# lgleznah/mort

Measured on AMD Instinct MI355X. Metric: Msamples/sec (width x height x spp/s), Scene 1 1200x675, higher is better.
Workload: dtype f32; 1 GPU; Scene 1 (random-spheres cover) 1200x675, 500 spp nominal = 484 effective, depth 20, megakernel, seed 69420, host LCG scene; mode=mega, partition=rows/8 interleaved over 1 rank(s)

## Files before the change

### mort_amd/csrc/hip/dev_scene.h

```cpp
#ifndef MORT_DEV_SCENE_H
#define MORT_DEV_SCENE_H

#include <stdint.h>
#include "mort_scene.h"

#define DREF(type, idx) (((uint32_t)(type) << 16) | (uint32_t)(idx))
#define DREF_TYPE(r) ((int)((r) >> 16) & 0x7fff)
#define DREF_IDX(r) ((int)((r) & 0xffffu))

struct __attribute__((aligned(16))) DSphere {
    float cx, cy, cz, radius;
    float vx, vy, vz;
    uint32_t mat;
};

struct __attribute__((aligned(16))) DQuad {
    float Q[3], D;
    float u[3], area;
    float v[3]; uint32_t mat;
    float n[3]; uint32_t pad0;
    float w[3]; uint32_t pad1;
};

struct __attribute__((aligned(16))) DBvhNode {
    float xmin, xmax, ymin, ymax, zmin, zmax;
    uint32_t skip;
    uint32_t prims;
};

struct __attribute__((aligned(16))) DNode2 {
    float x0min, x0max, y0min, y0max;
    float z0min, z0max, x1min, x1max;
    float y1min, y1max, z1min, z1max;
    uint32_t child0, child1;
    float e0, e1;
};
struct __attribute__((aligned(16))) DNode4 {
    float xmin[4], xmax[4], ymin[4], ymax[4], zmin[4], zmax[4], e[4];
    uint32_t child[4];
    uint32_t pad[4];
};
struct __attribute__((aligned(16))) DLeaf2 {
    DSphere a, b;
    float xmin, xmax, ymin, ymax, zmin, zmax;
    uint32_t n;
    uint32_t prims;
    uint32_t pad[4];
};
#define MORT_NODE4_PIECES 9
#define MORT_LEAF2_PIECES 7
#define MORT_OWN4_STACK 24
struct __attribute__((aligned(16))) DNodeQ {
    float ox, oy, oz;
    uint32_t exps;
    uint32_t q0;
    uint32_t q1;
    uint32_t q2;
    uint32_t children;
};
#define GLEAF_FIRST(ref) ((ref) & 0x1fffu)
#define GLEAF_COUNT(ref) ((((ref) >> 13) & 3u) + 1u)
#define MORT_OWN_STACK 16
#define MORT_OWN_MAX_DEPTH 15
#ifndef MORT_GEN_LEAF_MAX
#define MORT_GEN_LEAF_MAX 2
#endif
#define GENT(kind, chain, idx) (((uint32_t)(kind) << 31) | ((uint32_t)(chain) << 24) | (uint32_t)(idx))
#define GENT_QUAD(e) ((e) >> 31)
#define GENT_CHAIN(e) (((e) >> 24) & 0x7fu)
#define GENT_IDX(e) ((e) & 0xffffffu)

enum { XF_TRANSLATE = 0, XF_ROTATE_Y = 1 };
// ... 47 lines not shown
```

### mort_amd/csrc/hip/mega_bvh.h

```cpp
#ifndef MORT_MEGA_BVH_H
#define MORT_MEGA_BVH_H

#include "dev_render.h"


struct FastArgs {
    RenderArgs r;
    const unsigned char *hot_src;
    uint32_t hot_bytes;
    uint32_t off_nodes4, off_leafrecs, off_lambert, off_metal, off_diel, off_dlight, off_iso, off_solid, off_checker;
    uint32_t off_tstack;
    int node_first, node_count;
    unsigned int *next_q;
    int tiles_x, tiles_total;
    uint32_t off_stack;
    int stack_lds_depth;
    const unsigned *tile_order;
    int gen_tiles;
    int spread_shift;
    unsigned *tile_cost;
    int th_s, th_l, t_keep;
    int sub;
    float *vaccum;
    float4 *deep;
// ... 12 lines not shown
#define MORT_BVH_ARG_NAME
#endif
#ifdef MORT_BVH_NO_PIN
#define BU_I(x) (x)
#define BU_U(x) (x)
#define BU_F(x) (x)
#define BU_P(x) (x)
#else
#define BU_I(x) uni_i(x)
#define BU_U(x) uni_u(x)
#define BU_F(x) uni_f(x)
#define BU_P(x) uni_p(x)
#endif
__device__ __forceinline__ int uni_i(int x) { return __builtin_amdgcn_readfirstlane(x); }
__device__ __forceinline__ uint32_t uni_u(uint32_t x) { return (uint32_t)__builtin_amdgcn_readfirstlane((int)x); }
__device__ __forceinline__ float uni_f(float x) { return __int_as_float(__builtin_amdgcn_readfirstlane(__float_as_int(x))); }
template <typename T> __device__ __forceinline__ T *uni_p(T *p) {
    const unsigned long long v = (unsigned long long)p;
    const uint32_t lo = uni_u((uint32_t)v), hi = uni_u((uint32_t)(v >> 32));
    return (T *)(((unsigned long long)hi << 32) | (unsigned long long)lo);
}

enum { ST_T = 0, ST_L = 1, ST_S = 2, ST_DONE = 3 };
enum { FL_TIE = 1, FL_REF = 2 };
#ifdef MORT_REGION_MARKS
#define REGION(name) asm volatile("; REGION " name)
#else
#define REGION(name) do { } while (0)
#endif

DEV bool own_inv_ok(float v) { const float a = mort_fabsf(v); return a > 1e-15f && a < 1e15f; }
struct V3Ret { float x, y, z; };
__device__ __attribute__((noinline)) V3Ret texture_value_uv(const DScene *sc, uint32_t tex, float nx, float ny, float nz, float px, float py, float pz) {
    float u, v;
    sphere_uv(mk(nx, ny, nz), u, v);
    const V3 c = texture_value(*sc, tex, u, v, mk(px, py, pz));
    V3Ret r; r.x = c.x; r.y = c.y; r.z = c.z;
    return r;
}

struct RefHit { int best; float closest; };
__device__ __attribute__((noinline)) RefHit reference_walk(const DBvhNode *nodes, int node_first, int node_end, const DSphere *spheres,
                                                           float ox, float oy, float oz, float dx, float dy, float dz, float tm, float ray_a) {
    Ray ray; ray.o = mk(ox, oy, oz); ray.d = mk(dx, dy, dz); ray.tm = tm;
    float closest = __builtin_inff();
    int best = -1;
    const double dix = 1.0 / (double)ray.d.x, diy = 1.0 / (double)ray.d.y, diz = 1.0 / (double)ray.d.z;
// ... 25 lines not shown
    const float sqrtd = mort_sqrtf(discriminant);
    float root = (-half_b - sqrtd) / a;
    if (root < t_min || t_max < root) {
        root = (-half_b + sqrtd) / a;
        if (root < t_min || t_max < root) return -1.0f;
    }
    return root;
}

struct OwnRay { float ix, iy, iz, mx, my, mz, band, invlen; };

DEV bool own_prune(float xmin, float xmax, float ymin, float ymax, float zmin, float zmax, float e, const OwnRay &r, float closest, float &te_out) {
    const float px0 = __builtin_fmaf(xmin, r.ix, -r.mx), px1 = __builtin_fmaf(xmax, r.ix, -r.mx);
    const float py0 = __builtin_fmaf(ymin, r.iy, -r.my), py1 = __builtin_fmaf(ymax, r.iy, -r.my);
    const float pz0 = __builtin_fmaf(zmin, r.iz, -r.mz), pz1 = __builtin_fmaf(zmax, r.iz, -r.mz);
    const float te = __builtin_fmaxf(__builtin_fmaxf(__builtin_fminf(px0, px1), __builtin_fminf(py0, py1)),
                                     __builtin_fmaxf(__builtin_fminf(pz0, pz1), 0.001f));
    const float tx = __builtin_fminf(__builtin_fminf(__builtin_fmaxf(px0, px1), __builtin_fmaxf(py0, py1)), __builtin_fmaxf(pz0, pz1));
    const float tau = __builtin_fmaf(__builtin_fmaxf(mort_fabsf(te), mort_fabsf(tx)), 9.5367431640625e-07f, r.band);
    const float key = __builtin_fmaf(te, 0.992f, -__builtin_fmaf(e, r.invlen, tau));
    te_out = te;
    return (tx - te < -tau) || (key > closest);
}

typedef float v2f_t __attribute__((ext_vector_type(2)));
DEV void own_prune2(v2f_t xmin, v2f_t xmax, v2f_t ymin, v2f_t ymax, v2f_t zmin, v2f_t zmax, v2f_t e, const OwnRay &r, float closest,
                    float &te_a, float &te_b, bool &skip_a, bool &skip_b) {
    const v2f_t ix = {r.ix, r.ix}, iy = {r.iy, r.iy}, iz = {r.iz, r.iz};
    const v2f_t nmx = {-r.mx, -r.mx}, nmy = {-r.my, -r.my}, nmz = {-r.mz, -r.mz};
    const v2f_t px0 = __builtin_elementwise_fma(xmin, ix, nmx), px1 = __builtin_elementwise_fma(xmax, ix, nmx);
    const v2f_t py0 = __builtin_elementwise_fma(ymin, iy, nmy), py1 = __builtin_elementwise_fma(ymax, iy, nmy);
    const v2f_t pz0 = __builtin_elementwise_fma(zmin, iz, nmz), pz1 = __builtin_elementwise_fma(zmax, iz, nmz);
    v2f_t te, tx;
    te.x = __builtin_fmaxf(__builtin_fmaxf(__builtin_fminf(px0.x, px1.x), __builtin_fminf(py0.x, py1.x)), __builtin_fmaxf(__builtin_fminf(pz0.x, pz1.x), 0.001f));
    te.y = __builtin_fmaxf(__builtin_fmaxf(__builtin_fminf(px0.y, px1.y), __builtin_fminf(py0.y, py1.y)), __builtin_fmaxf(__builtin_fminf(pz0.y, pz1.y), 0.001f));
    tx.x = __builtin_fminf(__builtin_fminf(__builtin_fmaxf(px0.x, px1.x), __builtin_fmaxf(py0.x, py1.x)), __builtin_fmaxf(pz0.x, pz1.x));
    tx.y = __builtin_fminf(__builtin_fminf(__builtin_fmaxf(px0.y, px1.y), __builtin_fmaxf(py0.y, py1.y)), __builtin_fmaxf(pz0.y, pz1.y));
    v2f_t am;
    am.x = __builtin_fmaxf(mort_fabsf(te.x), mort_fabsf(tx.x)); am.y = __builtin_fmaxf(mort_fabsf(te.y), mort_fabsf(tx.y));
    const v2f_t c20 = {9.5367431640625e-07f, 9.5367431640625e-07f}, band = {r.band, r.band}, il = {r.invlen, r.invlen}, c992 = {0.992f, 0.992f};
    const v2f_t tau = __builtin_elementwise_fma(am, c20, band);
    const v2f_t key = __builtin_elementwise_fma(te, c992, -__builtin_elementwise_fma(e, il, tau));
    const v2f_t gap = tx - te;
    te_a = te.x; te_b = te.y;
    skip_a = (gap.x < -tau.x) || (key.x > closest);
    skip_b = (gap.y < -tau.y) || (key.y > closest);
// ... 10 lines not shown
    const float m = __builtin_fmaxf(__builtin_fmaxf(__builtin_fmaxf(mort_fabsf(px0), mort_fabsf(px1)), __builtin_fmaxf(mort_fabsf(py0), mort_fabsf(py1))),
                                    __builtin_fmaxf(mort_fabsf(pz0), mort_fabsf(pz1)));
    const float gap = t_max - t_min;
    const bool decided = (mort_fabsf(gap) > m * 9.5367431640625e-07f) && (m < 1e30f) && (m > 1e-30f);
    bool hit = gap > 0;
    if (!decided) hit = slab_exact(nd, ray.o.x, ray.o.y, ray.o.z, 1.0 / (double)ray.d.x, 1.0 / (double)ray.d.y, 1.0 / (double)ray.d.z, closest);
    return hit;
}
enum { K_SHADE = 0, K_FINISH = 1, K_NEWSAMPLE = 2, K_NEWPIX = 3 };

#ifndef MORT_TH_S
#define MORT_TH_S 48
#endif
#ifndef MORT_TH_L
#define MORT_TH_L 16
#endif
#ifndef MORT_T_UNROLL
#define MORT_T_UNROLL 1
#endif
#ifndef MORT_T_KEEP
#define MORT_T_KEEP 16
#endif

#ifndef MORT_MIN_WAVES
#define MORT_MIN_WAVES 3
#endif
#ifndef MORT_FAST_BLOCK
#define MORT_FAST_BLOCK 768
#endif

template <bool PROBE, bool SUB = false>
__device__ __attribute__((noinline)) void pixel_write(const FastArgs *fap, float sx, float sy, float sz, int lofs, uint32_t segments,
                                                      uint32_t draws, uint32_t d, uint32_t v0, uint32_t v1, uint32_t v2, uint32_t v3, uint32_t v4) {
    const FastArgs &fa = *fap;
    const RenderArgs &a = fa.r;
    if (SUB) {
        fa.vaccum[3 * (size_t)lofs] = sx; fa.vaccum[3 * (size_t)lofs + 1] = sy; fa.vaccum[3 * (size_t)lofs + 2] = sz;
        mort_rng_state st;
        st.d = d; st.v[0] = v0; st.v[1] = v1; st.v[2] = v2; st.v[3] = v3; st.v[4] = v4;
        st.boxmuller_flag = 0; st.boxmuller_flag_double = 0; st.boxmuller_extra = 0.f; st.boxmuller_extra_double = 0.;
        a.states[lofs] = st;
        const unsigned slot = 32u + 2u * (blockIdx.x & 31u);
        atomicAdd(&a.counters[slot], (unsigned long long)segments);
        atomicAdd(&a.counters[slot + 1u], (unsigned long long)draws);
        return;
    }
// ... 123 lines not shown
    const FastArgs &s_fa = fa_byval;
#else
    __shared__ FastArgs s_fa;
    const FastArgs *const fap = (const FastArgs *)__builtin_amdgcn_kernarg_segment_ptr();
    {
        const uint32_t *src = (const uint32_t *)fap;
        uint32_t *dst = (uint32_t *)&s_fa;
        for (uint32_t i = threadIdx.x; i < (uint32_t)(sizeof(FastArgs) / 4); i += BLOCK) dst[i] = src[i];
    }
#endif
    {
        const uint4 *src = (const uint4 *)fap->hot_src;
        uint4 *dst = (uint4 *)lds;
        const uint32_t n16 = fap->hot_bytes >> 4;
        for (uint32_t i = threadIdx.x; i < n16; i += BLOCK) dst[i] = src[i];
    }
    __syncthreads();
    if (threadIdx.x == 0) cam_view_fill(s_cam, s_fa.r);
    __syncthreads();
    const FastArgs &L = s_fa;
    static_assert(sizeof(DNode4) == 16 * MORT_NODE4_PIECES && sizeof(DLeaf2) == 16 * MORT_LEAF2_PIECES, "record strides");
    const float4 *nodes4 = (const float4 *)(lds + BU_U(L.off_nodes4));
    const float4 *leafrecs = (const float4 *)(lds + BU_U(L.off_leafrecs));
    const uint32_t ts_base = BU_U(L.off_tstack) + 2u * threadIdx.x;
#define TS_AT(off) (*(unsigned short *)(lds + (off)))
    const DLambert *lambert = (const DLambert *)(lds + BU_U(L.off_lambert));
    const DMetal *metal = (const DMetal *)(lds + BU_U(L.off_metal));
    const DDielectric *dielectric = (const DDielectric *)(lds + BU_U(L.off_diel));
    const DLambert *dlight = (const DLambert *)(lds + BU_U(L.off_dlight));
    const DLambert *isotropic = (const DLambert *)(lds + BU_U(L.off_iso));
    const DSolid *solid = (const DSolid *)(lds + BU_U(L.off_solid));
    const DChecker *checker = (const DChecker *)(lds + BU_U(L.off_checker));

    const int node_first = BU_I(L.node_first), node_end = node_first + BU_I(L.node_count);
    const int th_s = BU_I(L.th_s), th_l = BU_I(L.th_l), t_keep = BU_I(L.t_keep);
    const int sqrt_spp = BU_I(L.r.sqrt_spp), bounce_limit = BU_I(L.r.bounce_limit);
    const float bg_x = BU_F(L.r.background.x), bg_y = BU_F(L.r.background.y), bg_z = BU_F(L.r.background.z);
    const int spp = sqrt_spp * sqrt_spp;
    const unsigned total_q = (unsigned)BU_I(L.tiles_total) * 64u;

    int state = ((int)(threadIdx.x & 63u) < BU_I(L.lane_cap)) ? ST_S : ST_DONE, kind = K_NEWPIX;
    int xy = 0, lofs = 0;
    Rng rng; rng.d = rng.v0 = rng.v1 = rng.v2 = rng.v3 = rng.v4 = 0; rng.draws = 0;
    V3 pixel_color = mk(0, 0, 0);
    int s_ij = 0, iter = 0;
    uint32_t segments = 0;
    Ray ray; ray.o = mk(0, 0, 0); ray.d = mk(0, 0, 1); ray.tm = 0;
    float ray_time0 = 0;
    OwnRay orr; orr.ix = orr.iy = orr.iz = 1; orr.mx = orr.my = orr.mz = 0; orr.band = 0; orr.invlen = 1;
    float ray_a = 1, closest = 0;
    int best = -1;
    uint32_t node = 0;
    uint32_t spa = ts_base;
    int flags = 0;
    float4 *stack_deep = BU_P(L.deep) + ((size_t)blockIdx.x * BLOCK + threadIdx.x);
    const size_t deep_stride = (size_t)gridDim.x * BLOCK;
    unsigned long long ident_mask = 0ull;
    float4 *stack_lds = (float4 *)(lds + BU_U(L.off_stack));
    const int DL = BU_I(L.stack_lds_depth);
#ifdef MORT_PROFILE_STATES
    unsigned long long *const counters_p = fap->r.counters;
    unsigned long long prof[6] = {0, 0, 0, 0, 0, 0};
    unsigned long long prof_truns = 0;
    unsigned long long profc[8] = {0, 0, 0, 0, 0, 0, 0, 0};
    unsigned long long ps0 = 0, ps1;
#define PROFS0() do { ps0 = __builtin_readcyclecounter(); } while (0)
#define PROFS(i) do { ps1 = __builtin_readcyclecounter(); profc[i] += ps1 - ps0; ps0 = ps1; } while (0)
    unsigned long long pt0 = __builtin_readcyclecounter(), pt1;
    const unsigned long long prof_r0 = __builtin_amdgcn_s_memrealtime();
#define PROF(i, lanes) do { prof[2 * (i)] += 1; prof[2 * (i) + 1] += (unsigned long long)(lanes); } while (0)
    unsigned long long profb[12] = {0, 0, 0, 0, 0, 0, 0, 0, 0, 0, 0, 0};
#ifdef MORT_PROFILE_FINE
#define PROFB(i) do { } while (0)
    unsigned long long proff[12] = {0, 0, 0, 0, 0, 0, 0, 0, 0, 0, 0, 0};
#define PROFF(i) do { ps1 = __builtin_readcyclecounter(); proff[i] += ps1 - ps0; profc[4] += ps1 - ps0; ps0 = ps1; } while (0)
#else
// ... 30 lines not shown
        if (nS >= e_s) pick = ST_S;
        else if (nL >= e_l) pick = ST_L;
        else if (nT > 0) pick = ST_T;
        else pick = (nL >= nS) ? ST_L : ST_S;
        if (DRAIN && leader >= 0) {
            if (drain_rounds) pick = nT > 0 ? ST_T : nL > 0 ? ST_L : ST_S;
            else { const int ls = __builtin_amdgcn_readlane(state, leader); if (ls <= ST_S) pick = ls; }
        }
        PROFC(3);

                REGION("T");
        if (pick != ST_T && pick != ST_L) break;
        if (pick == ST_T) {
            int keep;
#ifdef MORT_PROFILE_STATES
            prof_truns++;
#endif
            do {
#pragma unroll
                for (int rep = 0; rep < MORT_T_UNROLL; rep++) {
                PROF(0, __popcll(__ballot(state == ST_T)));
                if (state == ST_T) {
                    const float4 *np = nodes4 + node;
                    const float4 bx0 = np[0], bx1 = np[1], by0 = np[2], by1 = np[3], bz0 = np[4], bz1 = np[5], be = np[6];
                    const uint4 ch = ((const uint4 *)np)[7];
                    float t0, t1, t2, t3;
#ifdef MORT_BVH_PACKED_FMA
                    bool m0, m1, m2, m3;
                    own_prune2(v2f_t{bx0.x, bx0.y}, v2f_t{bx1.x, bx1.y}, v2f_t{by0.x, by0.y}, v2f_t{by1.x, by1.y}, v2f_t{bz0.x, bz0.y}, v2f_t{bz1.x, bz1.y}, v2f_t{be.x, be.y}, orr, closest, t0, t1, m0, m1);
                    own_prune2(v2f_t{bx0.z, bx0.w}, v2f_t{bx1.z, bx1.w}, v2f_t{by0.z, by0.w}, v2f_t{by1.z, by1.w}, v2f_t{bz0.z, bz0.w}, v2f_t{bz1.z, bz1.w}, v2f_t{be.z, be.w}, orr, closest, t2, t3, m2, m3);
                    m2 = m2 || ch.z == 0xffffu; m3 = m3 || ch.w == 0xffffu;
#else
                    const bool m0 = own_prune(bx0.x, bx1.x, by0.x, by1.x, bz0.x, bz1.x, be.x, orr, closest, t0);
                    const bool m1 = own_prune(bx0.y, bx1.y, by0.y, by1.y, bz0.y, bz1.y, be.y, orr, closest, t1);
                    const bool m2 = own_prune(bx0.z, bx1.z, by0.z, by1.z, bz0.z, bz1.z, be.z, orr, closest, t2) || ch.z == 0xffffu;
                    const bool m3 = own_prune(bx0.w, bx1.w, by0.w, by1.w, bz0.w, bz1.w, be.w, orr, closest, t3) || ch.w == 0xffffu;
#endif
                    uint32_t k0 = m0 ? 0xffffffffu : ((__float_as_uint(t0) & 0xffff0000u) | ch.x);
                    uint32_t k1 = m1 ? 0xffffffffu : ((__float_as_uint(t1) & 0xffff0000u) | ch.y);
                    uint32_t k2 = m2 ? 0xffffffffu : ((__float_as_uint(t2) & 0xffff0000u) | ch.z);
                    uint32_t k3 = m3 ? 0xffffffffu : ((__float_as_uint(t3) & 0xffff0000u) | ch.w);
#define MORT_CSWAP(a, b) do { const uint32_t lo_ = a < b ? a : b, hi_ = a < b ? b : a; a = lo_; b = hi_; } while (0)
                    MORT_CSWAP(k0, k1); MORT_CSWAP(k2, k3); MORT_CSWAP(k0, k2); MORT_CSWAP(k1, k3); MORT_CSWAP(k1, k2);
#undef MORT_CSWAP
                    if (k3 != 0xffffffffu) { TS_AT(spa) = (unsigned short)k3; spa += 2u * BLOCK; }
                    if (k2 != 0xffffffffu) { TS_AT(spa) = (unsigned short)k2; spa += 2u * BLOCK; }
                    if (k1 != 0xffffffffu) { TS_AT(spa) = (unsigned short)k1; spa += 2u * BLOCK; }
                    uint32_t next = k0;
                    const bool none = k0 == 0xffffffffu;
                    const bool have = !none || spa != ts_base;
                    if (none && spa != ts_base) { spa -= 2u * BLOCK; next = TS_AT(spa); }
                    if (!have) { state = ST_S; kind = K_SHADE; }
                    else { node = next & 0x7fffu; if (next & 0x8000u) state = ST_L; }
                }
                }
                keep = __popcll(__ballot(state == ST_T));
                if (DRAIN && leader >= 0) keep = drain_rounds ? (keep > 0 ? 64 : 0) : (__builtin_amdgcn_readlane(state, leader) == ST_T) ? 64 : 0;
                else if (keep > 0 && keep < t_keep) {
                    const int wL = __popcll(__ballot(state == ST_L)), wS = __popcll(__ballot(state == ST_S));
                    if (!(wS >= e_s || wL >= e_l)) keep = 64;
                }
            } while (keep >= t_keep);
            PROFC(0);
        }
        if (pick == ST_L) {
                REGION("L");
            PROF(1, nL);
            if (state == ST_L) {
                const float4 *lp = leafrecs + node;
                const float4 a0 = lp[0], a1 = lp[1], b0 = lp[2], b1 = lp[3];
                const uint32_t two = ((const uint4 *)lp)[5].z;
                DSphere sa, sb;
                sa.cx = a0.x; sa.cy = a0.y; sa.cz = a0.z; sa.radius = a0.w; sa.vx = a1.x; sa.vy = a1.y; sa.vz = a1.z; sa.mat = __float_as_uint(a1.w);
                sb.cx = b0.x; sb.cy = b0.y; sb.cz = b0.z; sb.radius = b0.w; sb.vx = b1.x; sb.vy = b1.y; sb.vz = b1.z; sb.mat = __float_as_uint(b1.w);
                const float ta = sphere_hit_root(sa, ray, ray_a, 0.001f, closest);
                if (ta != -1.0f) {
                    if (ta == closest && best >= 0) flags |= FL_TIE;
                    closest = ta; best = (int)(node << 16);
                }
                if (two == 2u) {
                    const float tb = sphere_hit_root(sb, ray, ray_a, 0.001f, closest);
                    if (tb != -1.0f) {
                        if (tb == closest && best >= 0) flags |= FL_TIE;
                        closest = tb; best = (int)((node << 16) | 0x8000u);
                    }
                }
                if (spa != ts_base) {
                    spa -= 2u * BLOCK;
                    const uint32_t next = TS_AT(spa);
                    node = next & 0x7fffu;
                    state = (next & 0x8000u) ? ST_L : ST_T;
                } else { state = ST_S; kind = K_SHADE; }
            }
            PROFC(1);
        }
      }
      if (!running) break;
        {
            PROF(2, nS);
            PROFS0();
            V3 final_value = mk(0, 0, 0);
                REGION("S:verify");
            if (state == ST_S) {
                if (kind == K_SHADE) {
                    bool need_ref = flags != 0;
                    if (!need_ref && best >= 0) {
                        const float4 *lp = leafrecs + (best >> 16);
                        const float4 b0 = lp[4], b1 = lp[5];
                        DBvhNode lb;
                        lb.xmin = b0.x; lb.xmax = b0.y; lb.ymin = b0.z; lb.ymax = b0.w; lb.zmin = b1.x; lb.zmax = b1.y; lb.skip = 0; lb.prims = 0;
                        need_ref = !slab_check(lb, ray, orr, closest);
                    }
                    if (need_ref) {
                        atomicAdd(&fap->r.counters[3], 1ull);
                        const RefHit h = reference_walk(fap->r.sc.nodes, node_first, node_end, fap->r.sc.spheres, ray.o.x, ray.o.y, ray.o.z,
                                                        ray.d.x, ray.d.y, ray.d.z, ray.tm, ray_a);
                        best = h.best; closest = h.closest;
                    }
                    PROFF(0);
                REGION("S:hitrecord");
                    if (best < 0) {
                        final_value = mk(bg_x, bg_y, bg_z);
                        kind = K_FINISH;
                    } else {
                        DSphere sp;
                        if (need_ref) sp = fap->r.sc.spheres[best];
                        else {
                            const float4 *lp = leafrecs + (best >> 16) + ((best & 0x8000) ? 2 : 0);
// ... 159 lines not shown
                REGION("S:getray");
                PROFS(6);
                if (state != ST_DONE) {
                    if (kind == K_NEWSAMPLE) {
                        PROFB(4);
                        ray = get_ray(s_cam, xy & 0xffff, (xy >> 16) & 0x7fff, rng, s_ij & 0xffff, s_ij >> 16);
                        ray_time0 = ray.tm;
                        iter = 0;
                        kind = K_SHADE;
                        if (bounce_limit <= 0) { final_value = mk(0, 0, 0); kind = K_FINISH; }
                    }
                REGION("S:setup");
                    if (kind == K_SHADE) {
                        ray_a = vlen2(ray.d);
                        orr.ix = 1.0f / ray.d.x; orr.iy = 1.0f / ray.d.y; orr.iz = 1.0f / ray.d.z;
                        orr.mx = ray.o.x * orr.ix; orr.my = ray.o.y * orr.iy; orr.mz = ray.o.z * orr.iz;
                        const float mm = __builtin_fmaxf(__builtin_fmaxf(mort_fabsf(orr.mx), mort_fabsf(orr.my)), mort_fabsf(orr.mz));
                        orr.band = mm * 4.76837158203125e-07f;
                        orr.invlen = 1.01f / mort_sqrtf(ray_a);
                        const bool ordinary = own_inv_ok(orr.ix) && own_inv_ok(orr.iy) && own_inv_ok(orr.iz) && (mm < 1e30f);
                        closest = __builtin_inff();
                        best = -1;
                        node = 0; spa = ts_base;
                        flags = ordinary ? 0 : FL_REF;
                        segments++;
                        state = ordinary ? ST_T : ST_S;
                    }
                }
            }
                REGION("S:end");
            if (DRAIN && __ballot(state == ST_DONE) != 0ull) {
                unsigned key = (state <= ST_S) ? ((unsigned)((s_ij >> 16) * sqrt_spp + (s_ij & 0xffff)) << 6) | (threadIdx.x & 63u) : 0xffffffffu;
                for (int off = 32; off > 0; off >>= 1) { const unsigned o = (unsigned)__shfl_xor((int)key, off); key = o < key ? o : key; }
                leader = (key == 0xffffffffu) ? -1 : __builtin_amdgcn_readfirstlane((int)(key & 63u));
            }
            PROFS(7);
            PROFC(2);
        }
    }
    if ((threadIdx.x & 63) == 0) {
#ifdef MORT_PROFILE_STATES
#ifdef MORT_PROFILE_FINE
        for (int k = 0; k < 12; k++) atomicAdd(&counters_p[18 + k], proff[k]);
#endif
        for (int k = 0; k < 6; k++) atomicAdd(&counters_p[4 + k], prof[k]);
        atomicAdd(&counters_p[30], prof_truns);
        for (int k = 0; k < 4; k++) atomicAdd(&counters_p[10 + k], profc[k]);
// ... 13 lines not shown
```

### mort_amd/csrc/hip/mort_hip.hip

```cpp
#include <hip/hip_runtime.h>

#include <algorithm>
#include <climits>
#include <cmath>
#include <cstdio>
#include <cstdlib>
#include <cstring>
#include <new>
#include <string>
#include <vector>

#include "mort_hip.h"
#include "dev_pixel.h"
#include "scene_blob.h"
#include "seed_host.h"
#include "mort_internal.h"
#include "mort_ctx.h"
#include "mega_gen.h"
#include "wave_gen.h"

#pragma clang fp contract(off)


#ifndef MORT_GENERIC_WAVES
#define MORT_GENERIC_WAVES 4
#endif
#ifndef MORT_MEGA_LDS_LEVELS
#define MORT_MEGA_LDS_LEVELS 9
#endif
extern "C" __global__ void __launch_bounds__(256, MORT_GENERIC_WAVES)
mega_kernel(const RenderArgs a) {
    const int lane = threadIdx.x & 63;
// ... 533 lines not shown
    return FB == 1024 ? mega_bvh_kernel<1024, false, false, true> : FB == 768 ? mega_bvh_kernel<768, false, false, true> : FB == 512 ? mega_bvh_kernel<512, false, false, true>
           : FB == 384 ? mega_bvh_kernel<384, false, false, true> : mega_bvh_kernel<256, false, false, true>;
}

static int launch_bvh(mort_ctx *c, const mort_camera *cam, const RenderArgs &a, int tiles, bool sub, bool timed, hipStream_t s, LaunchPlan &plan) {
    FastArgs fa;
    std::memset(&fa, 0, sizeof fa);
    fast_args_base(c, cam, a, fa, c->d_fast, c->fast_bytes, tiles, sub);
    fa.off_nodes4 = c->f_nodes4; fa.off_leafrecs = c->f_leafrecs; fa.off_lambert = c->f_lambert; fa.off_metal = c->f_metal;
    fa.off_diel = c->f_diel; fa.off_dlight = c->f_dlight; fa.off_iso = c->f_iso; fa.off_solid = c->f_solid; fa.off_checker = c->f_checker;
    fa.node_first = 0; fa.node_count = c->sc.n_nodes;
    const long long lanes_wanted = (long long)tiles * 64;
    const double px_per_lane = (double)lanes_wanted / ((double)c->num_cus * 768.0);
    int FB = MORT_FAST_BLOCK;
    const char *fb_env = std::getenv("MORT_FAST_BLOCK_SIZE");
    if (fb_env) FB = std::atoi(fb_env);
    else {
        const int cand[4] = {768, 512, 384, 256};
        FB = 256;
        const bool wide_ok = lanes_wanted >= 2ll * 1024 * c->num_cus;
        for (int k = (px_per_lane < 1.5 && !sub) ? 1 : 0; k < 4; k++) if (lanes_wanted >= (long long)cand[k] * c->num_cus) { FB = cand[k]; break; }
        if (wide_ok) FB = 1024;
    }
    if (FB == 1024 && (size_t)((fa.hot_bytes + 15u) & ~15u) + (size_t)c->own4_stack * 1024u * 2u + 2048u + 1024u * 16u > 160u * 1024u) FB = 768;
    if (FB != 1024 && FB != 768 && FB != 512 && FB != 384) FB = 256;
    fa.drain_rounds = 3;
    { const char *dm = std::getenv("MORT_BVH_DRAIN"); if (dm) fa.drain_rounds = std::atoi(dm) == 2 ? 1 : std::atoi(dm) == 3 ? 3 : 0; }
    bool chain_bound = px_per_lane < 1.5 && !sub;
    { const char *cb = std::getenv("MORT_CHAIN_BOUND"); if (cb && !sub) chain_bound = cb[0] == '1'; }
    if (FB == 1024) chain_bound = false;
    const bvh_kernel_t kern = bvh_kernel(FB, false, chain_bound, sub), kern_probe = bvh_kernel(FB, true, false, false);
    fa.th_s = MORT_TH_S; fa.th_l = MORT_TH_L; fa.t_keep = MORT_T_KEEP;
    { const char *th = std::getenv("MORT_THRESHOLDS");
      if (th) { int s_ = 0, l_ = 0, k_ = 0; if (std::sscanf(th, "%d,%d,%d", &s_, &l_, &k_) == 3 && s_ >= 1 && l_ >= 1 && k_ >= 1) { fa.th_s = s_; fa.th_l = l_; fa.t_keep = k_; } } }
    int per_cu_cap = INT_MAX;
    { const char *pc = std::getenv("MORT_FAST_BLOCKS_PER_CU"); if (pc && std::atoi(pc) >= 1) per_cu_cap = std::atoi(pc); }
    size_t lds_bytes = 0;
    int grid = 0;
    int st = state_setup(c, cam, fa, (const void *)kern, FB, (uint32_t)c->own4_stack, 12, per_cu_cap, "BVH image does not fit one CU's LDS", s, lds_bytes, grid);
    if (st != MORT_OK) return st;
    st = prepare_tile_order(c, cam, a, fa, tiles, grid, FB, chain_bound, sub, timed, s, [&](const FastArgs &pa) {
        hipError_t e_ = hipFuncSetAttribute((const void *)kern_probe, hipFuncAttributeMaxDynamicSharedMemorySize, (int)lds_bytes);
        if (e_ != hipSuccess) return e_;
        hipLaunchKernelGGL(kern_probe, dim3(grid), dim3(FB), lds_bytes, s, pa);
        return hipGetLastError();
    });
    if (st != MORT_OK) return st;
    hipLaunchKernelGGL(kern, dim3(grid), dim3(FB), lds_bytes, s, fa);
    HIPCHK(c, hipGetLastError());
    plan.kernel = (const void *)kern; plan.block = FB; plan.lds_bytes = (int)lds_bytes;
    std::snprintf(plan.name, sizeof plan.name, "mega_bvh_kernel<%d, false, %s, %s>", FB, chain_bound ? "true" : "false", sub ? "true" : "false");
    return MORT_OK;
}

static int launch_gen(mort_ctx *c, const mort_camera *cam, const RenderArgs &a, int tiles, bool sub, bool timed, hipStream_t s, LaunchPlan &plan) {
    GenArgs ga = c->gen;
    FastArgs &fa = ga.f;
    fast_args_base(c, cam, a, fa, c->d_gen, c->gen_bytes, tiles, sub);
    const long long lanes_wanted = (long long)tiles * 64;
    int FB = 768;
    bool heavy_default = false;
    { const char *fb_env = std::getenv("MORT_GEN_BLOCK_SIZE");
// ... 247 lines not shown
    const mortc::Compiled &o = sb.comp;
    for (int i = 0; i < 9; i++) out[i] = 0;
    out[0] = (int)o.own_nodes.size(); out[1] = (int)o.own_leaves.size(); out[2] = o.own_depth;
    out[3] = (int)o.own_nodes4.size(); out[4] = o.own4_stack;
    if (o.own_nodes4.empty()) return MORT_OK;
    struct Rec { float v[7]; };
    std::vector<Rec> of_inner(o.own_nodes.size()), of_leaf(o.own_leaves.size());
    for (const DNode2 &nd : o.own_nodes)
        for (int k = 0; k < 2; k++) {
            const uint32_t ref = k ? nd.child1 : nd.child0;
            Rec r = k ? Rec{{nd.x1min, nd.x1max, nd.y1min, nd.y1max, nd.z1min, nd.z1max, nd.e1}} : Rec{{nd.x0min, nd.x0max, nd.y0min, nd.y0max, nd.z0min, nd.z0max, nd.e0}};
            if (ref & 0x8000u) of_leaf[ref & 0x7fffu] = r; else of_inner[ref] = r;
        }
    std::vector<int> seen(o.own_leaves.size(), 0);
    std::vector<uint32_t> todo(1, 0u);
    bool same = true;
    while (!todo.empty()) {
        const uint32_t n = todo.back(); todo.pop_back();
        const DNode4 &nd = o.own_nodes4[n];
        for (int k = 0; k < 4; k++) {
            const uint32_t ref = nd.child[k];
            if (ref == 0xffffu) continue;
            out[7]++;
            const Rec r{{nd.xmin[k], nd.xmax[k], nd.ymin[k], nd.ymax[k], nd.zmin[k], nd.zmax[k], nd.e[k]}};
            if (ref & 0x8000u) {
                const uint32_t l = (ref & 0x7fffu) / MORT_LEAF2_PIECES;
                if ((ref & 0x7fffu) % MORT_LEAF2_PIECES || l >= seen.size() || seen[l]++) { out[6]++; continue; }
                out[5]++;
                if (std::memcmp(&r, &of_leaf[l], sizeof r) != 0) same = false;
            } else {
                if (ref % MORT_NODE4_PIECES || ref / MORT_NODE4_PIECES >= o.own_nodes4.size()) { out[6]++; continue; }
                bool found = false;
                for (const Rec &b : of_inner) if (std::memcmp(&r, &b, sizeof r) == 0) { found = true; break; }
                if (!found) same = false;
                todo.push_back(ref / MORT_NODE4_PIECES);
            }
        }
    }
    out[8] = same ? 1 : 0;
    return MORT_OK;
}

extern "C" int mort_hip_render_device(mort_ctx *c, const mort_camera *cam, int mode, void *d_rgba, void *d_accum,
                                      void *stream, mort_stats *stats) {
    return render_device_impl(c, cam, mode, d_rgba, d_accum, nullptr, stream, stats);
}

extern "C" int mort_hip_render(mort_ctx *c, const mort_camera *cam, int mode, uint8_t *rgba_out, float *accum_out,
                               uint32_t *segments_px_out, mort_stats *stats) {
    if (!c || !cam || !rgba_out) return MORT_ERR_INVALID;
    const int W = cam->image_width, H = cam->image_height;
    if (W <= 0 || H <= 0) return MORT_ERR_INVALID;
    HIPCHK(c, hipSetDevice(c->device));
    const int lr = local_rows_for(c->part, H);
    const size_t npx = (size_t)W * (size_t)lr;
    int st;
    if ((st = ensure_buf(c, &c->d_rgba, &c->rgba_cap, npx * 4)) != MORT_OK) return st;
    if (accum_out && (st = ensure_buf(c, &c->d_accum, &c->accum_cap, npx * 12)) != MORT_OK) return st;
    if (segments_px_out) { if ((st = ensure_buf(c, &c->d_segpx, &c->segpx_cap, npx * 4)) != MORT_OK) return st; }
    else if (c->d_segpx) { hipFree(c->d_segpx); c->d_segpx = nullptr; c->segpx_cap = 0; }
    mort_stats local;
    st = render_device_impl(c, cam, mode, c->d_rgba, accum_out ? c->d_accum : nullptr,
// ... 18 lines not shown
```

### mort_amd/csrc/hip/scene_compile.h

```cpp
#ifndef MORT_SCENE_COMPILE_H
#define MORT_SCENE_COMPILE_H

#include <algorithm>
#include <cmath>
#include <cstdlib>
#include <cstring>
#include <vector>

#include "dev_scene.h"
#include "mort_hip.h"

namespace mortc {

static const int kMaxChain = 8;
static const int kMaxDepth = 16;

struct Ref { int kind; int idx; int cf, cc; };

struct Compiled {
    std::vector<DItem> items, subitems;
    std::vector<DBvhNode> nodes;
    std::vector<DSphere> spheres, wspheres;
    std::vector<DQuad> quads, wquads;
    std::vector<DXform> xforms;
// ... 298 lines not shown
        s.ref = k ? nd.child1 : nd.child0; s.e = k ? nd.e1 : nd.e0;
        s.lo[0] = k ? nd.x1min : nd.x0min; s.hi[0] = k ? nd.x1max : nd.x0max;
        s.lo[1] = k ? nd.y1min : nd.y0min; s.hi[1] = k ? nd.y1max : nd.y0max;
        s.lo[2] = k ? nd.z1min : nd.z0min; s.hi[2] = k ? nd.z1max : nd.z0max;
        return s;
    }
    struct Cut4 { double t[5]; unsigned char left[5]; };
    void cut_expand(const std::vector<Cut4> &dp, const Slot4 &s, int k, std::vector<Slot4> &outv) const {
        if ((s.ref & 0x8000u) || dp[s.ref].left[k] == 0) { outv.push_back(s); return; }
        const int i = dp[s.ref].left[k];
        cut_expand(dp, slot_of(out.own_nodes[s.ref], 0), i, outv);
        cut_expand(dp, slot_of(out.own_nodes[s.ref], 1), k - i, outv);
    }
    int collapse_emit(const std::vector<Cut4> &dp, uint32_t b2, uint32_t me) {
        std::vector<Slot4> sl;
        const int i0 = dp[b2].left[0];
        cut_expand(dp, slot_of(out.own_nodes[b2], 0), i0, sl);
        cut_expand(dp, slot_of(out.own_nodes[b2], 1), 4 - i0, sl);
        int below = 0;
        DNode4 n4;
        std::memset(&n4, 0, sizeof n4);
        for (int k = 0; k < 4; k++) n4.child[k] = 0xffffu;
        for (size_t i = 0; i < sl.size() && i < 4; i++) {
            n4.xmin[i] = sl[i].lo[0]; n4.xmax[i] = sl[i].hi[0]; n4.ymin[i] = sl[i].lo[1]; n4.ymax[i] = sl[i].hi[1];
            n4.zmin[i] = sl[i].lo[2]; n4.zmax[i] = sl[i].hi[2]; n4.e[i] = sl[i].e;
            if (sl[i].ref & 0x8000u) { n4.child[i] = 0x8000u | ((sl[i].ref & 0x7fffu) * MORT_LEAF2_PIECES); continue; }
            const uint32_t ci = (uint32_t)out.own_nodes4.size();
            out.own_nodes4.push_back(DNode4{});
            n4.child[i] = ci * MORT_NODE4_PIECES;
            const int d = collapse_emit(dp, sl[i].ref, ci);
            if (d > below) below = d;
        }
        out.own_nodes4[me] = n4;
        return (int)sl.size() - 1 + below;
    }
    void collapse_own_tree() {
        out.own_nodes4.clear(); out.own4_stack = 0;
        const size_t n2 = out.own_nodes.size();
        if (n2 == 0) return;
        std::vector<double> area(n2, 0.0);
        {
            const Slot4 a = slot_of(out.own_nodes[0], 0), b = slot_of(out.own_nodes[0], 1);
            Box u; for (int k = 0; k < 3; k++) { u.lo[k] = std::fmin(a.lo[k], b.lo[k]); u.hi[k] = std::fmax(a.hi[k], b.hi[k]); }
            area[0] = box_area(u);
        }
        for (size_t n = 0; n < n2; n++)
            for (int k = 0; k < 2; k++) {
                const Slot4 c = slot_of(out.own_nodes[n], k);
// ... 374 lines not shown
```

Baseline: 3980 Msamples/s.

## Store duplicated min/max planes in BVH4 nodes for sign-ordered slab tests

The 4-wide BVH node layout becomes x[3][4], y[3][4], z[3][4] with the min plane duplicated after the max plane. Per-ray direction signs are packed into the flags word as byte offsets, so the traversal loads near and far planes directly and drops the per-axis min/max ops in the slab test. This trades a larger node record (11 vs 9 float4 pieces) and more LDS footprint for fewer ALU ops per box test. The LDS traversal stack also moves to pointer arithmetic, and an optional branch-free push variant plus host-side debug functions are added.

```diff
diff --git a/mort_amd/csrc/hip/dev_scene.h b/mort_amd/csrc/hip/dev_scene.h
--- a/mort_amd/csrc/hip/dev_scene.h
+++ b/mort_amd/csrc/hip/dev_scene.h
@@ -36,10 +36,14 @@
     float e0, e1;
 };
 struct __attribute__((aligned(16))) DNode4 {
-    float xmin[4], xmax[4], ymin[4], ymax[4], zmin[4], zmax[4], e[4];
+    float x[3][4], y[3][4], z[3][4], e[4];
     uint32_t child[4];
-    uint32_t pad[4];
 };
+#define MORT_NODE4_X 0
+#define MORT_NODE4_Y 3
+#define MORT_NODE4_Z 6
+#define MORT_NODE4_E 9
+#define MORT_NODE4_CHILD 10
 struct __attribute__((aligned(16))) DLeaf2 {
     DSphere a, b;
     float xmin, xmax, ymin, ymax, zmin, zmax;
@@ -47,7 +51,7 @@
     uint32_t prims;
     uint32_t pad[4];
 };
-#define MORT_NODE4_PIECES 9
+#define MORT_NODE4_PIECES 11
 #define MORT_LEAF2_PIECES 7
 #define MORT_OWN4_STACK 24
 struct __attribute__((aligned(16))) DNodeQ {
diff --git a/mort_amd/csrc/hip/mega_bvh.h b/mort_amd/csrc/hip/mega_bvh.h
--- a/mort_amd/csrc/hip/mega_bvh.h
+++ b/mort_amd/csrc/hip/mega_bvh.h
@@ -58,7 +58,8 @@
 }
 
 enum { ST_T = 0, ST_L = 1, ST_S = 2, ST_DONE = 3 };
-enum { FL_TIE = 1, FL_REF = 2 };
+enum { FL_TIE = 1, FL_REF = 2, FL_MASK = 3 };
+#define FL_SIGNS(ox, oy, oz) (int)(((ox) << 8) | ((oy) << 16) | ((oz) << 24))
 #ifdef MORT_REGION_MARKS
 #define REGION(name) asm volatile("; REGION " name)
 #else
@@ -130,6 +131,19 @@
     te_out = te;
     return (tx - te < -tau) || (key > closest);
 }
+
+DEV bool own_prune_ordered(float xn, float xf, float yn, float yf, float zn, float zf, float e, const OwnRay &r, float closest, float &te_out) {
+    const float pxn = __builtin_fmaf(xn, r.ix, -r.mx), pxf = __builtin_fmaf(xf, r.ix, -r.mx);
+    const float pyn = __builtin_fmaf(yn, r.iy, -r.my), pyf = __builtin_fmaf(yf, r.iy, -r.my);
+    const float pzn = __builtin_fmaf(zn, r.iz, -r.mz), pzf = __builtin_fmaf(zf, r.iz, -r.mz);
+    const float te = __builtin_fmaxf(__builtin_fmaxf(pxn, pyn), __builtin_fmaxf(pzn, 0.001f));
+    const float tx = __builtin_fminf(__builtin_fminf(pxf, pyf), pzf);
+    const float tau = __builtin_fmaf(__builtin_fmaxf(mort_fabsf(te), mort_fabsf(tx)), 9.5367431640625e-07f, r.band);
+    const float key = __builtin_fmaf(te, 0.992f, -__builtin_fmaf(e, r.invlen, tau));
+    te_out = te;
+    return (tx - te < -tau) || (key > closest);
+}
+DEV uint32_t own_sign_offset(float inv) { return (__builtin_bit_cast(uint32_t, inv) >> 27) & 16u; }
 
 typedef float v2f_t __attribute__((ext_vector_type(2)));
 DEV void own_prune2(v2f_t xmin, v2f_t xmax, v2f_t ymin, v2f_t ymax, v2f_t zmin, v2f_t zmax, v2f_t e, const OwnRay &r, float closest,
@@ -186,6 +200,11 @@
 #define MORT_T_KEEP 16
 #endif
 
+#ifdef MORT_BVH_PUSH_BRANCHFREE
+#define MORT_BVH_TSTACK_SPARE 1u
+#else
+#define MORT_BVH_TSTACK_SPARE 0u
+#endif
 #ifndef MORT_MIN_WAVES
 #define MORT_MIN_WAVES 3
 #endif
@@ -355,8 +374,8 @@
     static_assert(sizeof(DNode4) == 16 * MORT_NODE4_PIECES && sizeof(DLeaf2) == 16 * MORT_LEAF2_PIECES, "record strides");
     const float4 *nodes4 = (const float4 *)(lds + BU_U(L.off_nodes4));
     const float4 *leafrecs = (const float4 *)(lds + BU_U(L.off_leafrecs));
-    const uint32_t ts_base = BU_U(L.off_tstack) + 2u * threadIdx.x;
-#define TS_AT(off) (*(unsigned short *)(lds + (off)))
+    unsigned short *const ts_base = (unsigned short *)(lds + BU_U(L.off_tstack)) + threadIdx.x;
+#define TS_AT(ptr) (*(ptr))
     const DLambert *lambert = (const DLambert *)(lds + BU_U(L.off_lambert));
     const DMetal *metal = (const DMetal *)(lds + BU_U(L.off_metal));
     const DDielectric *dielectric = (const DDielectric *)(lds + BU_U(L.off_diel));
@@ -384,7 +403,7 @@
     float ray_a = 1, closest = 0;
     int best = -1;
     uint32_t node = 0;
-    uint32_t spa = ts_base;
+    unsigned short *spa = ts_base;
     int flags = 0;
     float4 *stack_deep = BU_P(L.deep) + ((size_t)blockIdx.x * BLOCK + threadIdx.x);
     const size_t deep_stride = (size_t)gridDim.x * BLOCK;
@@ -461,19 +480,26 @@
                 PROF(0, __popcll(__ballot(state == ST_T)));
                 if (state == ST_T) {
                     const float4 *np = nodes4 + node;
-                    const float4 bx0 = np[0], bx1 = np[1], by0 = np[2], by1 = np[3], bz0 = np[4], bz1 = np[5], be = np[6];
-                    const uint4 ch = ((const uint4 *)np)[7];
                     float t0, t1, t2, t3;
 #ifdef MORT_BVH_PACKED_FMA
+                    const float4 bx0 = np[MORT_NODE4_X], bx1 = np[MORT_NODE4_X + 1], by0 = np[MORT_NODE4_Y], by1 = np[MORT_NODE4_Y + 1];
+                    const float4 bz0 = np[MORT_NODE4_Z], bz1 = np[MORT_NODE4_Z + 1], be = np[MORT_NODE4_E];
+                    const uint4 ch = ((const uint4 *)np)[MORT_NODE4_CHILD];
                     bool m0, m1, m2, m3;
                     own_prune2(v2f_t{bx0.x, bx0.y}, v2f_t{bx1.x, bx1.y}, v2f_t{by0.x, by0.y}, v2f_t{by1.x, by1.y}, v2f_t{bz0.x, bz0.y}, v2f_t{bz1.x, bz1.y}, v2f_t{be.x, be.y}, orr, closest, t0, t1, m0, m1);
                     own_prune2(v2f_t{bx0.z, bx0.w}, v2f_t{bx1.z, bx1.w}, v2f_t{by0.z, by0.w}, v2f_t{by1.z, by1.w}, v2f_t{bz0.z, bz0.w}, v2f_t{bz1.z, bz1.w}, v2f_t{be.z, be.w}, orr, closest, t2, t3, m2, m3);
                     m2 = m2 || ch.z == 0xffffu; m3 = m3 || ch.w == 0xffffu;
 #else
-                    const bool m0 = own_prune(bx0.x, bx1.x, by0.x, by1.x, bz0.x, bz1.x, be.x, orr, closest, t0);
-                    const bool m1 = own_prune(bx0.y, bx1.y, by0.y, by1.y, bz0.y, bz1.y, be.y, orr, closest, t1);
-                    const bool m2 = own_prune(bx0.z, bx1.z, by0.z, by1.z, bz0.z, bz1.z, be.z, orr, closest, t2) || ch.z == 0xffffu;
-                    const bool m3 = own_prune(bx0.w, bx1.w, by0.w, by1.w, bz0.w, bz1.w, be.w, orr, closest, t3) || ch.w == 0xffffu;
+                    const unsigned char *nb = (const unsigned char *)np;
+                    const float4 *ax = (const float4 *)(nb + (((uint32_t)flags >> 8) & 0xffu)) + MORT_NODE4_X;
+                    const float4 *ay = (const float4 *)(nb + (((uint32_t)flags >> 16) & 0xffu)) + MORT_NODE4_Y;
+                    const float4 *az = (const float4 *)(nb + ((uint32_t)flags >> 24)) + MORT_NODE4_Z;
+                    const float4 xn = ax[0], xf = ax[1], yn = ay[0], yf = ay[1], zn = az[0], zf = az[1], be = np[MORT_NODE4_E];
+                    const uint4 ch = ((const uint4 *)np)[MORT_NODE4_CHILD];
+                    const bool m0 = own_prune_ordered(xn.x, xf.x, yn.x, yf.x, zn.x, zf.x, be.x, orr, closest, t0);
+                    const bool m1 = own_prune_ordered(xn.y, xf.y, yn.y, yf.y, zn.y, zf.y, be.y, orr, closest, t1);
+                    const bool m2 = own_prune_ordered(xn.z, xf.z, yn.z, yf.z, zn.z, zf.z, be.z, orr, closest, t2) || ch.z == 0xffffu;
+                    const bool m3 = own_prune_ordered(xn.w, xf.w, yn.w, yf.w, zn.w, zf.w, be.w, orr, closest, t3) || ch.w == 0xffffu;
 #endif
                     uint32_t k0 = m0 ? 0xffffffffu : ((__float_as_uint(t0) & 0xffff0000u) | ch.x);
                     uint32_t k1 = m1 ? 0xffffffffu : ((__float_as_uint(t1) & 0xffff0000u) | ch.y);
@@ -482,13 +508,19 @@
 #define MORT_CSWAP(a, b) do { const uint32_t lo_ = a < b ? a : b, hi_ = a < b ? b : a; a = lo_; b = hi_; } while (0)
                     MORT_CSWAP(k0, k1); MORT_CSWAP(k2, k3); MORT_CSWAP(k0, k2); MORT_CSWAP(k1, k3); MORT_CSWAP(k1, k2);
 #undef MORT_CSWAP
-                    if (k3 != 0xffffffffu) { TS_AT(spa) = (unsigned short)k3; spa += 2u * BLOCK; }
-                    if (k2 != 0xffffffffu) { TS_AT(spa) = (unsigned short)k2; spa += 2u * BLOCK; }
-                    if (k1 != 0xffffffffu) { TS_AT(spa) = (unsigned short)k1; spa += 2u * BLOCK; }
+#ifdef MORT_BVH_PUSH_BRANCHFREE
+                    TS_AT(spa) = (unsigned short)k3; spa += (k3 != 0xffffffffu) ? BLOCK : 0;
+                    TS_AT(spa) = (unsigned short)k2; spa += (k2 != 0xffffffffu) ? BLOCK : 0;
+                    TS_AT(spa) = (unsigned short)k1; spa += (k1 != 0xffffffffu) ? BLOCK : 0;
+#else
+                    if (k3 != 0xffffffffu) { TS_AT(spa) = (unsigned short)k3; spa += BLOCK; }
+                    if (k2 != 0xffffffffu) { TS_AT(spa) = (unsigned short)k2; spa += BLOCK; }
+                    if (k1 != 0xffffffffu) { TS_AT(spa) = (unsigned short)k1; spa += BLOCK; }
+#endif
                     uint32_t next = k0;
                     const bool none = k0 == 0xffffffffu;
                     const bool have = !none || spa != ts_base;
-                    if (none && spa != ts_base) { spa -= 2u * BLOCK; next = TS_AT(spa); }
+                    if (none && spa != ts_base) { spa -= BLOCK; next = TS_AT(spa); }
                     if (!have) { state = ST_S; kind = K_SHADE; }
                     else { node = next & 0x7fffu; if (next & 0x8000u) state = ST_L; }
                 }
@@ -525,7 +557,7 @@
                     }
                 }
                 if (spa != ts_base) {
-                    spa -= 2u * BLOCK;
+                    spa -= BLOCK;
                     const uint32_t next = TS_AT(spa);
                     node = next & 0x7fffu;
                     state = (next & 0x8000u) ? ST_L : ST_T;
@@ -542,7 +574,7 @@
                 REGION("S:verify");
             if (state == ST_S) {
                 if (kind == K_SHADE) {
-                    bool need_ref = flags != 0;
+                    bool need_ref = (flags & FL_MASK) != 0;
                     if (!need_ref && best >= 0) {
                         const float4 *lp = leafrecs + (best >> 16);
                         const float4 b0 = lp[4], b1 = lp[5];
@@ -748,7 +780,7 @@
                         closest = __builtin_inff();
                         best = -1;
                         node = 0; spa = ts_base;
-                        flags = ordinary ? 0 : FL_REF;
+                        flags = ordinary ? FL_SIGNS(own_sign_offset(orr.ix), own_sign_offset(orr.iy), own_sign_offset(orr.iz)) : FL_REF;
                         segments++;
                         state = ordinary ? ST_T : ST_S;
                     }
diff --git a/mort_amd/csrc/hip/mort_hip.hip b/mort_amd/csrc/hip/mort_hip.hip
--- a/mort_amd/csrc/hip/mort_hip.hip
+++ b/mort_amd/csrc/hip/mort_hip.hip
@@ -1,6 +1,7 @@
 #include <hip/hip_runtime.h>
 
 #include <algorithm>
+#include <array>
 #include <climits>
 #include <cmath>
 #include <cstdio>
@@ -8,6 +9,7 @@
 #include <cstring>
 #include <new>
 #include <string>
+#include <thread>
 #include <vector>
 
 #include "mort_hip.h"
@@ -587,7 +589,7 @@
         for (int k = (px_per_lane < 1.5 && !sub) ? 1 : 0; k < 4; k++) if (lanes_wanted >= (long long)cand[k] * c->num_cus) { FB = cand[k]; break; }
         if (wide_ok) FB = 1024;
     }
-    if (FB == 1024 && (size_t)((fa.hot_bytes + 15u) & ~15u) + (size_t)c->own4_stack * 1024u * 2u + 2048u + 1024u * 16u > 160u * 1024u) FB = 768;
+    if (FB == 1024 && (size_t)((fa.hot_bytes + 15u) & ~15u) + ((size_t)c->own4_stack + MORT_BVH_TSTACK_SPARE) * 1024u * 2u + 2048u + 1024u * 16u > 160u * 1024u) FB = 768;
     if (FB != 1024 && FB != 768 && FB != 512 && FB != 384) FB = 256;
     fa.drain_rounds = 3;
     { const char *dm = std::getenv("MORT_BVH_DRAIN"); if (dm) fa.drain_rounds = std::atoi(dm) == 2 ? 1 : std::atoi(dm) == 3 ? 3 : 0; }
@@ -602,7 +604,7 @@
     { const char *pc = std::getenv("MORT_FAST_BLOCKS_PER_CU"); if (pc && std::atoi(pc) >= 1) per_cu_cap = std::atoi(pc); }
     size_t lds_bytes = 0;
     int grid = 0;
-    int st = state_setup(c, cam, fa, (const void *)kern, FB, (uint32_t)c->own4_stack, 12, per_cu_cap, "BVH image does not fit one CU's LDS", s, lds_bytes, grid);
+    int st = state_setup(c, cam, fa, (const void *)kern, FB, (uint32_t)c->own4_stack + MORT_BVH_TSTACK_SPARE, 12, per_cu_cap, "BVH image does not fit one CU's LDS", s, lds_bytes, grid);
     if (st != MORT_OK) return st;
     st = prepare_tile_order(c, cam, a, fa, tiles, grid, FB, chain_bound, sub, timed, s, [&](const FastArgs &pa) {
         hipError_t e_ = hipFuncSetAttribute((const void *)kern_probe, hipFuncAttributeMaxDynamicSharedMemorySize, (int)lds_bytes);
@@ -896,7 +898,8 @@
             const uint32_t ref = nd.child[k];
             if (ref == 0xffffu) continue;
             out[7]++;
-            const Rec r{{nd.xmin[k], nd.xmax[k], nd.ymin[k], nd.ymax[k], nd.zmin[k], nd.zmax[k], nd.e[k]}};
+            const Rec r{{nd.x[0][k], nd.x[1][k], nd.y[0][k], nd.y[1][k], nd.z[0][k], nd.z[1][k], nd.e[k]}};
+            if (std::memcmp(&nd.x[2][k], &nd.x[0][k], 4) || std::memcmp(&nd.y[2][k], &nd.y[0][k], 4) || std::memcmp(&nd.z[2][k], &nd.z[0][k], 4)) same = false;
             if (ref & 0x8000u) {
                 const uint32_t l = (ref & 0x7fffu) / MORT_LEAF2_PIECES;
                 if ((ref & 0x7fffu) % MORT_LEAF2_PIECES || l >= seen.size() || seen[l]++) { out[6]++; continue; }
@@ -912,6 +915,78 @@
         }
     }
     out[8] = same ? 1 : 0;
+    return MORT_OK;
+}
+
+extern "C" int mort_hip_debug_own_tree4_boxes(const mort_world *w, float *out, size_t max_boxes) {
+    if (!w || (!out && max_boxes)) return MORT_ERR_INVALID;
+    SceneBlob sb;
+    const int st = build_scene_blob(w, sb);
+    if (st != MORT_OK) return st;
+    size_t n = 0;
+    for (const DNode4 &nd : sb.comp.own_nodes4)
+        for (int k = 0; k < 4; k++) {
+            if (nd.child[k] == 0xffffu) continue;
+            if (n < max_boxes) { float *o = out + 6 * n; o[0] = nd.x[0][k]; o[1] = nd.x[1][k]; o[2] = nd.y[0][k]; o[3] = nd.y[1][k]; o[4] = nd.z[0][k]; o[5] = nd.z[1][k]; }
+            n++;
+        }
+    return (int)n;
+}
+
+extern "C" int mort_hip_debug_prune_forms(const mort_world *w, const float *rays, size_t n, int stride, unsigned long long *out) {
+    if (!w || !rays || !out || stride < 1) return MORT_ERR_INVALID;
+    SceneBlob sb;
+    const int st = build_scene_blob(w, sb);
+    if (st != MORT_OK) return st;
+    const std::vector<DNode4> &nodes = sb.comp.own_nodes4;
+    for (int i = 0; i < 16; i++) out[i] = 0;
+    out[4] = nodes.size();
+    if (nodes.empty()) return MORT_OK;
+    for (const DNode4 &nd : nodes)
+        for (int k = 0; k < 4; k++) {
+            if (nd.child[k] != 0xffffu) continue;
+            const float v[10] = {nd.x[0][k], nd.x[1][k], nd.x[2][k], nd.y[0][k], nd.y[1][k], nd.y[2][k], nd.z[0][k], nd.z[1][k], nd.z[2][k], nd.e[k]};
+            for (float f : v) { uint32_t b; std::memcpy(&b, &f, 4); if (b) { out[5]++; break; } }
+        }
+    unsigned nthreads = std::thread::hardware_concurrency();
+    if (nthreads < 1) nthreads = 1;
+    if (nthreads > 16) nthreads = 16;
+    std::vector<std::array<unsigned long long, 16>> part(nthreads);
+    auto work = [&](unsigned t) {
+        std::array<unsigned long long, 16> &o = part[t];
+        o.fill(0);
+        for (size_t r = t; r < n; r += nthreads) {
+            const float *q = rays + 7 * r;
+            OwnRay orr;
+            orr.ix = 1.0f / q[3]; orr.iy = 1.0f / q[4]; orr.iz = 1.0f / q[5];
+            orr.mx = q[0] * orr.ix; orr.my = q[1] * orr.iy; orr.mz = q[2] * orr.iz;
+            const float mm = __builtin_fmaxf(__builtin_fmaxf(mort_fabsf(orr.mx), mort_fabsf(orr.my)), mort_fabsf(orr.mz));
+            orr.band = mm * 4.76837158203125e-07f;
+            orr.invlen = 1.01f / mort_sqrtf(q[3] * q[3] + q[4] * q[4] + q[5] * q[5]);
+            if (!(own_inv_ok(orr.ix) && own_inv_ok(orr.iy) && own_inv_ok(orr.iz) && (mm < 1e30f))) { o[3]++; continue; }
+            const uint32_t sx = own_sign_offset(orr.ix) / 16u, sy = own_sign_offset(orr.iy) / 16u, sz = own_sign_offset(orr.iz) / 16u;
+            o[8 + (sx | sy << 1 | sz << 2)]++;
+            const float closest = q[6];
+            for (size_t ni = r % (size_t)stride; ni < nodes.size(); ni += (size_t)stride) {
+                const DNode4 &nd = nodes[ni];
+                for (int k = 0; k < 4; k++) {
+                    if (nd.child[k] == 0xffffu) continue;
+                    float te_a, te_b;
+                    const bool skip_a = own_prune(nd.x[0][k], nd.x[1][k], nd.y[0][k], nd.y[1][k], nd.z[0][k], nd.z[1][k], nd.e[k], orr, closest, te_a);
+                    const bool skip_b = own_prune_ordered(nd.x[sx][k], nd.x[sx + 1][k], nd.y[sy][k], nd.y[sy + 1][k], nd.z[sz][k], nd.z[sz + 1][k], nd.e[k], orr, closest, te_b);
+                    o[0]++;
+                    if (std::memcmp(&te_a, &te_b, 4) != 0) o[1]++;
+                    if (skip_a != skip_b) o[2]++;
+                    if (skip_a && skip_b) o[6]++;
+                }
+            }
+        }
+    };
+    std::vector<std::thread> pool;
+    for (unsigned t = 1; t < nthreads; t++) pool.emplace_back(work, t);
+    work(0);
+    for (std::thread &th : pool) th.join();
+    for (const auto &o : part) for (int i = 0; i < 16; i++) if (i != 4 && i != 5) out[i] += o[i];
     return MORT_OK;
 }
 
diff --git a/mort_amd/csrc/hip/scene_compile.h b/mort_amd/csrc/hip/scene_compile.h
--- a/mort_amd/csrc/hip/scene_compile.h
+++ b/mort_amd/csrc/hip/scene_compile.h
@@ -344,8 +344,10 @@
         std::memset(&n4, 0, sizeof n4);
         for (int k = 0; k < 4; k++) n4.child[k] = 0xffffu;
         for (size_t i = 0; i < sl.size() && i < 4; i++) {
-            n4.xmin[i] = sl[i].lo[0]; n4.xmax[i] = sl[i].hi[0]; n4.ymin[i] = sl[i].lo[1]; n4.ymax[i] = sl[i].hi[1];
-            n4.zmin[i] = sl[i].lo[2]; n4.zmax[i] = sl[i].hi[2]; n4.e[i] = sl[i].e;
+            n4.x[0][i] = n4.x[2][i] = sl[i].lo[0]; n4.x[1][i] = sl[i].hi[0];
+            n4.y[0][i] = n4.y[2][i] = sl[i].lo[1]; n4.y[1][i] = sl[i].hi[1];
+            n4.z[0][i] = n4.z[2][i] = sl[i].lo[2]; n4.z[1][i] = sl[i].hi[2];
+            n4.e[i] = sl[i].e;
             if (sl[i].ref & 0x8000u) { n4.child[i] = 0x8000u | ((sl[i].ref & 0x7fffu) * MORT_LEAF2_PIECES); continue; }
             const uint32_t ci = (uint32_t)out.own_nodes4.size();
             out.own_nodes4.push_back(DNode4{});
```

After: 4246 Msamples/s (median of 6 runs). 1.07x the previous value.
